# cryscan/bevy-hikari

Hardware: NVIDIA H100
Metric: Mrays/s (higher is better)
Workload: dtype f32

## Files before the change

### bevy_hikari_b200/csrc/context.cu

```cuda
#include <cuda_runtime.h>
#ifndef HK_EMU
#include <cuda.h>
#endif
#include <math.h>
#include <stdio.h>
#include <stdlib.h>
#include <string.h>

#include <algorithm>
#include <array>
#include <set>
#include <string>
#include <unordered_set>
#include <vector>

#include "hikari_b200.h"
#include "hk_kernels.h"
#include "wide_build.h"

#ifndef HK_POOLED_INDIRECT
#define HK_POOLED_INDIRECT 0
#endif

#ifndef HK_WIDE_TRAVERSAL_DEFAULT
// ... 37 lines not shown
    std::vector<hk_node> host_asset_nodes;
    std::vector<uint32_t> host_primitive_vertex_index;
    std::set<std::array<uint32_t, 4>> mesh_range_checked;
    Planes planes{};
    DeviceScene scene{};
    bool scene_ready = false, noise_ready = false;
    bool planes_ready = false;
    TileMap tm_depth[2], tm_q3[2][2];
    TileMap tm_denoise[4][5];
    bool tile_maps_ready = false;
    bool full_frame = true;
    int last_up_w = 0, last_up_h = 0;
    bool last_scaled = false;
    int last_render_w = 0, last_render_h = 0; bool last_smaa = false, last_upscalers = false, last_fsr = false; uint32_t last_number = 0;
    int gbuffer_current = 0;
    uint8_t* noise = nullptr;
    Counters* counters = nullptr;
    SpatialTable* spatial_tables = nullptr;
    SpatialTable spatial_tables_host[2];
    bool count_rays = false, time_passes = false, keep_intermediates = false;
    bool pooled_indirect = HK_POOLED_INDIRECT != 0;
    bool tiled_denoise = true;
    bool tiled_spatial = true;
    int wide_traversal = 0;
    uint32_t wide_tlas_node_count = 0;
    cudaStream_t copy_stream = nullptr;
    cudaEvent_t ev_submitted = nullptr, ev_copied = nullptr;
    bool copy_in_flight = false;
    bool copy_unwaited = false;
    uint2* frame_target = nullptr; uint32_t frame_pitch = 0;
    bool tile_upscalers = false;
    int motion_margin = 0;
    std::vector<void*> frames_owned, frames_opened;
    std::vector<hk_halo_peer*> halo_peers;
    float trace_ms = 0.0f;
    cudaEvent_t ev[4] = {nullptr, nullptr, nullptr, nullptr};
    cudaEvent_t kev[HK_K_COUNT][2] = {};
    int time_only = -1;
    static const int RING = 256;
    cudaEvent_t ring[RING][2] = {};
    uint32_t ring_frames = 0;
    bool ring_hit = false;
    bool kran[HK_K_COUNT] = {};
    hk_frame_stats stats{};
    uint32_t launches = 0;
    std::string error;
// ... 65 lines not shown
    const uint64_t rows = (uint64_t)(b.a1 - b.a0), pitch = (uint64_t)b.AW;
    bool ok = true;
    for (int v = 0; v < 2 && ok; ++v) {
        const uint32_t bh = 16u + 2u * (v ? 10u : 20u), bw = (uint32_t)tile_box_width((int)bh);
        ok = make_tile_map(&ctx->tm_depth[v], ctx->planes.depth, 4, pitch, rows, pitch * 4, bw, bh);
        for (int parity = 0; parity < 2 && ok; ++parity)
            ok = make_tile_map(&ctx->tm_q3[v][parity], ctx->planes.reservoir[(v ? 2 : 6) + parity].q[3], 4, pitch * 4, rows, pitch * 16, bw * 4, bh);
    }
    for (int level = 0; level < 4 && ok; ++level) {
        const uint32_t step = 8u >> level, bh = 16u + 2u * step, bw = (uint32_t)tile_box_width((int)bh);
        ok = make_tile_map(&ctx->tm_denoise[level][0], ctx->planes.dn_geometry, 4, pitch * 4, rows, pitch * 16, bw * 4, bh) &&
             make_tile_map(&ctx->tm_denoise[level][1], ctx->planes.dn_instance, 4, pitch, rows, pitch * 4, bw, bh);
        for (int sgl = 0; sgl < 3 && ok; ++sgl)
            ok = make_tile_map(&ctx->tm_denoise[level][2 + sgl], ctx->planes.dn_internal[level][sgl], 4, pitch * 2, rows, pitch * 8, bw * 2, bh);
    }
    return ok;
}

static int allocate_planes(hk_context* ctx, uint32_t width, uint32_t height, uint32_t col_begin, uint32_t col_end,
                           uint32_t row_begin, uint32_t row_end) {
    if (width == 0 || height == 0 || row_begin >= row_end || row_end > height || col_begin >= col_end || col_end > width)
        return set_error(ctx, HK_ERR_INVALID_ARGUMENT, "bad size or tile rectangle");
    ctx->planes_ready = false;
    ctx->last_render_w = ctx->last_render_h = 0; ctx->last_up_w = ctx->last_up_h = 0; ctx->last_number = 0; ctx->last_scaled = false;
    ctx->last_smaa = ctx->last_upscalers = ctx->last_fsr = false;
    ctx->frame_target = nullptr; ctx->frame_pitch = 0;
    free_list(ctx->allocations);
    ctx->planes = Planes{};
    Band b;
    b.W = (int)width; b.H = (int)height; b.r0 = (int)row_begin; b.r1 = (int)row_end; b.cx0 = (int)col_begin; b.cx1 = (int)col_end;
    const int ghost = GHOST_TEMPORAL + ctx->motion_margin;
    b.a0 = b.r0 - ghost < 0 ? 0 : b.r0 - ghost;
    b.a1 = b.r1 + ghost > b.H ? b.H : b.r1 + ghost;
    b.ax0 = b.cx0 - ghost < 0 ? 0 : b.cx0 - ghost;
    b.ax1 = b.cx1 + ghost > b.W ? b.W : b.cx1 + ghost;
    b.AW = hk_plane_pitch(b.ax1 - b.ax0);
    b.RW = b.W; b.RH = b.H; b.RS = b.AW; b.OW = 2 * b.W; b.OH = 2 * b.H;
    ctx->band = b;
    const size_t n = (size_t)b.AW * (size_t)(b.a1 - b.a0);
    ctx->band_pixels = n;
    ctx->owned_pixels = (size_t)(b.cx1 - b.cx0) * (size_t)(b.r1 - b.r0);
    Planes& p = ctx->planes;
    auto& L = ctx->allocations;
    ctx->full_frame = (b.cx0 == 0 && b.cx1 == b.W && b.r0 == 0 && b.r1 == b.H);
    ctx->gbuffer_current = 0;
    HK_CUDA(alloc_plane(ctx, &p.pos_depth_db[0], n, L));
    HK_CUDA(alloc_plane(ctx, &p.pos_depth_db[1], n, L));
    HK_CUDA(alloc_plane(ctx, &p.velocity_uv_db[0], n, L));
    HK_CUDA(alloc_plane(ctx, &p.velocity_uv_db[1], n, L));
    p.pos_depth = p.pos_depth_db[0];
    p.velocity_uv = p.velocity_uv_db[0];
    HK_CUDA(alloc_plane(ctx, &p.depth, n, L));
    HK_CUDA(alloc_plane(ctx, &p.normal, n, L));
    HK_CUDA(alloc_plane(ctx, &p.depth_gradient, n, L));
    HK_CUDA(alloc_plane(ctx, &p.instance_material, n, L));
    HK_CUDA(alloc_plane(ctx, &p.albedo, n, L));
    HK_CUDA(alloc_plane(ctx, &p.dn_geometry, n, L));
    HK_CUDA(alloc_plane(ctx, &p.dn_instance, n, L));
    for (int i = 0; i < 3; ++i) {
        HK_CUDA(alloc_plane(ctx, &p.render[i], n, L));
        HK_CUDA(alloc_plane(ctx, &p.variance[i], n, L));
        HK_CUDA(alloc_plane(ctx, &p.dn_variance[i], n, L));
        HK_CUDA(alloc_plane(ctx, &p.dn_render[i], n, L));
        for (int l = 0; l < 4; ++l) HK_CUDA(alloc_plane(ctx, &p.dn_internal[l][i], n, L));
    }
    for (int r = 0; r < 10; ++r)
        for (int q = 0; q < 4; ++q) HK_CUDA(alloc_plane(ctx, &p.reservoir[r].q[q], n, L));
    HK_CUDA(alloc_plane(ctx, &p.scatter_key, n, L));
    for (int q = 0; q < 4; ++q) HK_CUDA(alloc_plane(ctx, &p.scatter_value.q[q], n, L));
    HK_CUDA(alloc_plane(ctx, &p.tone_mapped_db[0], ctx->owned_pixels, L));
    HK_CUDA(alloc_plane(ctx, &p.tone_mapped_db[1], ctx->owned_pixels, L));
    p.tone_mapped = p.tone_mapped_db[0];
    p.upscale_output = nullptr; p.upscale_sharpen_output = nullptr; p.taa_output[0] = p.taa_output[1] = nullptr;
    p.tone_ring_db[0] = p.tone_ring_db[1] = nullptr;
    if (!ctx->full_frame && ctx->tile_upscalers) {
// ... 19 lines not shown

int hk_context_create(hk_context** out, int cuda_device, uint32_t width, uint32_t height, uint32_t row_begin, uint32_t row_end,
                      void* cuda_stream) {
    return hk_context_create_tile(out, cuda_device, width, height, 0, width, row_begin, row_end, cuda_stream);
}

int hk_context_create_tile(hk_context** out, int cuda_device, uint32_t width, uint32_t height, uint32_t col_begin, uint32_t col_end,
                           uint32_t row_begin, uint32_t row_end, void* cuda_stream) {
    hk_context* ctx = nullptr;
    if (!out) return set_error(nullptr, HK_ERR_INVALID_ARGUMENT, "out == NULL");
    *out = nullptr;
    int ndev = 0;
    cudaError_t e = cudaGetDeviceCount(&ndev);
    if (e != cudaSuccess || ndev == 0)
        return set_error(nullptr, HK_ERR_CUDA, std::string("no CUDA device: ") + cudaGetErrorString(e) +
                                                   " (this library has no CPU fallback)");
    if (cuda_device < 0 || cuda_device >= ndev) return set_error(nullptr, HK_ERR_INVALID_ARGUMENT, "bad cuda_device");
    HK_CUDA(cudaSetDevice(cuda_device));
    hk_context* c = new hk_context();
    c->device = cuda_device;
    if (const char* e = getenv("HK_TUNE_POOLED_INDIRECT")) c->pooled_indirect = atoi(e) != 0;
    if (const char* e = getenv("HK_TUNE_TILED_SPATIAL")) c->tiled_spatial = atoi(e) != 0;
    if (const char* e = getenv("HK_TUNE_TILED_DENOISE")) c->tiled_denoise = atoi(e) != 0;
    c->wide_traversal = hk_tolerance_build() != 0 ? HK_WIDE_TRAVERSAL_DEFAULT : 0;
    if (const char* e = getenv("HK_TUNE_WIDE_TRAVERSAL")) c->wide_traversal = atoi(e) & 3;
#ifndef HK_EMU
    if (const char* e = getenv("HK_TUNE_PREFER_L1")) { if (atoi(e)) cudaDeviceSetCacheConfig(cudaFuncCachePreferL1); }
#endif
    ctx = c;
    if (cuda_stream) c->stream = reinterpret_cast<cudaStream_t>(cuda_stream);
    else {
        e = cudaStreamCreateWithFlags(&c->stream, cudaStreamNonBlocking);
        if (e != cudaSuccess) { delete c; return set_error(nullptr, HK_ERR_CUDA, cudaGetErrorString(e)); }
        c->own_stream = true;
    }
    int rc = allocate_planes(c, width, height, col_begin, col_end, row_begin, row_end);
    if (rc == HK_OK) {
        void* p = nullptr;
        if (cudaMalloc(&p, sizeof(Counters)) != cudaSuccess) rc = set_error(c, HK_ERR_OUT_OF_MEMORY, "counters");
        else { c->counters = reinterpret_cast<Counters*>(p); cudaMemsetAsync(p, 0, sizeof(Counters), c->stream); }
    }
    if (rc == HK_OK) {
        SpatialTable t[2];
        memset(t, 0, sizeof(t));
        for (int v = 0; v < 2; ++v) {
            const uint32_t count = v ? 8u : 16u;
// ... 568 lines not shown
                                                  "and a motion margin of at least 4 pixels + the per-frame motion");
    if (in->temporal_upscalers && in->fsr1 && in->smaa_tu4x)
        return set_error(ctx, HK_ERR_INVALID_ARGUMENT, "fsr1 and smaa_tu4x are the two variants of one enum (Upscale, lib.rs:475-490)");
    if (in->temporal_upscalers && in->fsr1 && !ctx->full_frame)
        return set_error(ctx, HK_ERR_UNSUPPORTED, "FSR1 needs a full-frame context (no tile)");
    if (in->frame.direct_validate_interval == 0 || in->frame.emissive_validate_interval == 0)
        return set_error(ctx, HK_ERR_INVALID_ARGUMENT, "validate interval must be >= 1");
    if (cudaSetDevice(ctx->device) != cudaSuccess) return set_error(ctx, HK_ERR_CUDA, "cudaSetDevice");
    P.in = *in;
    P.scene = ctx->scene;
    P.planes = ctx->planes;
    P.planes.pos_depth = ctx->planes.pos_depth_db[ctx->gbuffer_current];
    P.planes.velocity_uv = ctx->planes.velocity_uv_db[ctx->gbuffer_current];
    P.planes.tone_mapped = ctx->planes.tone_mapped_db[in->temporal_upscalers ? (in->frame.number % 2u) : 0u];
    ctx->last_upscalers = in->temporal_upscalers != 0;
    P.band = ctx->band;
    P.ratio1 = ratio1 ? 1 : 0;
    P.jitter_sign = ((in->frame.number & 1u) == 0u) ? -1.0f : 1.0f;
    P.ratio_m1 = in->frame.upscale_ratio - 1.0f;
    P.gbuffer_current = ctx->gbuffer_current;
    P.frame_target = ratio1 ? ctx->frame_target : nullptr;
    P.frame_pitch = ctx->frame_pitch;
    P.tile_images = (!ctx->full_frame && in->temporal_upscalers) ? 1 : 0;
    if (!ratio1) {
        const float scale = 1.0f / in->frame.upscale_ratio;
        P.band.RW = (int)ceilf(scale * (float)P.band.W);
        P.band.RH = (int)ceilf(scale * (float)P.band.H);
        P.band.RS = P.band.RW;
    }
    {
        const float scale2 = (1.0f / in->frame.upscale_ratio) * 2.0f;
        P.band.OW = (int)ceilf((float)P.band.W * scale2);
        P.band.OH = (int)ceilf((float)P.band.H * scale2);
    }
    ctx->last_up_w = P.band.OW; ctx->last_up_h = P.band.OH; ctx->last_scaled = !ratio1;
    P.inv_rw = 1.0f / (float)P.band.RW; P.inv_rh = 1.0f / (float)P.band.RH;
    ctx->last_render_w = P.band.RW; ctx->last_render_h = P.band.RH; ctx->last_smaa = in->smaa_tu4x != 0; ctx->last_number = in->frame.number;
    ctx->last_fsr = in->temporal_upscalers && in->fsr1;
    P.counters = ctx->count_rays ? ctx->counters : nullptr;
    P.noise = ctx->noise;
    float s, c;
    hk::sincos_(in->frame.solar_angle, &s, &c);
    P.cos_solar_angle = c;
    P.random_frame = hk::random_float(in->frame.number);
    P.spatial_tables = ctx->spatial_tables;
    return HK_OK;
// ... 35 lines not shown
}

struct KernelTimer {
    hk_context* c; int k;
    KernelTimer(hk_context* ctx, int kernel) : c(ctx), k(kernel) {
        c->launches += 1;
        if (c->time_only >= 0) {
            if (c->time_only == k && c->ring[0][0]) { cudaEventRecord(c->ring[c->ring_frames % hk_context::RING][0], c->stream); c->ring_hit = true; }
        } else if (c->time_passes) { cudaEventRecord(c->kev[k][0], c->stream); c->kran[k] = true; }
    }
    ~KernelTimer() {
        if (c->time_only >= 0) {
            if (c->time_only == k && c->ring[0][0]) cudaEventRecord(c->ring[c->ring_frames % hk_context::RING][1], c->stream);
        } else if (c->time_passes) cudaEventRecord(c->kev[k][1], c->stream);
    }
};

static int run_prepass(hk_context* ctx, KParams& P) {
    ctx->gbuffer_current ^= 1;
    P.gbuffer_current = ctx->gbuffer_current;
    P.planes.pos_depth = ctx->planes.pos_depth_db[ctx->gbuffer_current];
    P.planes.velocity_uv = ctx->planes.velocity_uv_db[ctx->gbuffer_current];
    rows_deferred(ctx, P, GHOST_TEMPORAL + ctx->motion_margin);
    { KernelTimer t(ctx, HK_K_GBUFFER); hk_launch_gbuffer(P, ctx->count_rays, wide_primary(ctx), ctx->stream); }
    return check_launch(ctx);
}
static int ring_of(const KParams& P) { return P.tile_images ? RING_TONE : 0; }
static void launch_spatial(hk_context* ctx, const KParams& P, bool emissive) {
    const int v = emissive ? 1 : 0, parity = 1 - (int)(P.in.frame.number & 1u);
    const bool tiled = ctx->tile_maps_ready && ctx->tiled_spatial;
    hk_launch_spatial(P, emissive, tiled ? &ctx->tm_depth[v] : nullptr, tiled ? &ctx->tm_q3[v][parity] : nullptr, ctx->spatial_tables_host[v], ctx->stream);
}
static const TileMap* denoise_maps(hk_context* ctx, int level) { return (ctx->tile_maps_ready && ctx->tiled_denoise) ? ctx->tm_denoise[level] : nullptr; }
static int run_light(hk_context* ctx, KParams& P) {
    const hk_frame_uniform& f = P.in.frame;
    const int GHOST_SPATIAL = ::GHOST_SPATIAL + ring_of(P);
    rows(ctx, P, GHOST_TEMPORAL + ctx->motion_margin);
    { KernelTimer t(ctx, HK_K_DIRECT); hk_launch_direct(P, false, ctx->count_rays, wide_light(ctx), ctx->stream);
      hk_launch_scatter_resolve(P, 0, ctx->stream); ctx->launches += 1; }
    { KernelTimer t(ctx, HK_K_EMISSIVE); hk_launch_direct(P, true, ctx->count_rays, wide_light(ctx), ctx->stream);
      hk_launch_scatter_resolve(P, 1, ctx->stream); ctx->launches += 1; }
    if (f.emissive_spatial_reuse) { rows(ctx, P, GHOST_SPATIAL); KernelTimer t(ctx, HK_K_EMISSIVE_SPATIAL); launch_spatial(ctx, P, true); }
    rows(ctx, P, GHOST_TEMPORAL + ctx->motion_margin);
    { KernelTimer t(ctx, HK_K_INDIRECT);
      if (ctx->pooled_indirect) hk_launch_indirect_pool(P, f.indirect_bounces >= 2, ctx->count_rays, ctx->stream);
      else hk_launch_indirect(P, f.indirect_bounces >= 2, ctx->count_rays, wide_light(ctx), ctx->stream);
      hk_launch_scatter_resolve(P, 2, ctx->stream); ctx->launches += 1; }
// ... 49 lines not shown
        }
    }
    return check_launch(ctx);
}

int hk_prepass_run(hk_context* ctx, const hk_frame_inputs* in) {
    KParams P; int rc = make_params(ctx, in, P); if (rc) return rc;
    ctx->launches = 0;
    return run_prepass(ctx, P);
}
int hk_import_gbuffer(hk_context* ctx, const hk_gbuffer_desc* g) {
    if (!ctx || !g) return HK_ERR_INVALID_ARGUMENT;
    if (!ctx->planes_ready) return set_error(ctx, HK_ERR_NOT_READY, "per-pixel planes are not allocated (a resize failed)");
    if (!g->position || !g->normal || !g->depth_gradient || !g->instance_material || !g->velocity_uv)
        return set_error(ctx, HK_ERR_INVALID_ARGUMENT, "hk_import_gbuffer: all five planes are required");
    const Band& b = ctx->band;
    const size_t ow = (size_t)(b.cx1 - b.cx0), oh = (size_t)(b.r1 - b.r0);
    const size_t pitch[5] = {g->position_pitch_bytes, g->normal_pitch_bytes, g->depth_gradient_pitch_bytes, g->instance_material_pitch_bytes, g->velocity_uv_pitch_bytes};
    const size_t bpp[5] = {16, 4, 8, 8, 16};
    for (int i = 0; i < 5; ++i)
        if (pitch[i] < ow * bpp[i]) return set_error(ctx, HK_ERR_INVALID_ARGUMENT, "hk_import_gbuffer: a row pitch is smaller than the owned rectangle's row");
    HK_CUDA(cudaSetDevice(ctx->device));
    ctx->gbuffer_current ^= 1;
    Planes& p = ctx->planes;
    const size_t first = (size_t)(b.r0 - b.a0) * (size_t)b.AW + (size_t)(b.cx0 - b.ax0);
    void* dst[5] = {p.pos_depth_db[ctx->gbuffer_current] + first, p.normal + first, p.depth_gradient + first, p.instance_material + first,
                    p.velocity_uv_db[ctx->gbuffer_current] + first};
    const void* src[5] = {g->position, g->normal, g->depth_gradient, g->instance_material, g->velocity_uv};
    for (int i = 0; i < 5; ++i)
        HK_CUDA(cudaMemcpy2DAsync(dst[i], (size_t)b.AW * bpp[i], src[i], pitch[i], ow * bpp[i], oh, cudaMemcpyDeviceToDevice, ctx->stream));
    return HK_OK;
}
int hk_light_run(hk_context* ctx, const hk_frame_inputs* in) {
    KParams P; int rc = make_params(ctx, in, P); if (rc) return rc;
    ctx->launches = 0;
    rows_deferred(ctx, P, GHOST_TEMPORAL + ctx->motion_margin);
    hk_launch_albedo(P, ctx->stream);
    ctx->launches += 1;
    return run_light(ctx, P);
}
int hk_post_process_run(hk_context* ctx, const hk_frame_inputs* in) {
    KParams P; int rc = make_params(ctx, in, P); if (rc) return rc;
    ctx->launches = 0;
    return run_post(ctx, P, false);
}
int hk_run_pass(hk_context* ctx, const hk_frame_inputs* in, int pass, int arg) {
// ... 46 lines not shown
    return HK_OK;
}

int hk_sync(hk_context* ctx) {
    if (!ctx) return HK_ERR_INVALID_ARGUMENT;
    HK_CUDA(cudaSetDevice(ctx->device));
    HK_CUDA(cudaStreamSynchronize(ctx->stream));
    if (ctx->copy_unwaited) { HK_CUDA(cudaEventSynchronize(ctx->ev_copied)); ctx->copy_unwaited = false; }
    return HK_OK;
}

int hk_set_profiling(hk_context* ctx, int count_rays, int time_passes) {
    if (!ctx) return HK_ERR_INVALID_ARGUMENT;
    ctx->count_rays = count_rays != 0;
    ctx->time_passes = time_passes != 0;
    return HK_OK;
}
int hk_set_tuning(hk_context* ctx, int key, int value) {
    if (!ctx) return HK_ERR_INVALID_ARGUMENT;
    switch (key) {
        case HK_TUNE_POOLED_INDIRECT: ctx->pooled_indirect = value != 0; return HK_OK;
        case HK_TUNE_TILED_SPATIAL: ctx->tiled_spatial = value != 0; return HK_OK;
        case HK_TUNE_TILED_DENOISE: ctx->tiled_denoise = value != 0; return HK_OK;
        case HK_TUNE_WIDE_TRAVERSAL:
            if (value < 0 || value > 3 || value == 2) return set_error(ctx, HK_ERR_INVALID_ARGUMENT, "HK_TUNE_WIDE_TRAVERSAL takes 0, 1 or 3");
            ctx->wide_traversal = value; return HK_OK;
        default: return set_error(ctx, HK_ERR_INVALID_ARGUMENT, "unknown tuning key");
    }
}
int hk_set_profiling_kernel(hk_context* ctx, int kernel) {
    if (!ctx || kernel >= HK_K_COUNT) return HK_ERR_INVALID_ARGUMENT;
    HK_CUDA(cudaSetDevice(ctx->device));
    ctx->time_only = kernel < 0 ? -1 : kernel;
    ctx->ring_frames = 0;
    if (kernel >= 0 && !ctx->ring[0][0])
        for (int i = 0; i < hk_context::RING; ++i)
            for (int j = 0; j < 2; ++j) HK_CUDA(cudaEventCreate(&ctx->ring[i][j]));
    return HK_OK;
}
int hk_set_keep_intermediates(hk_context* ctx, int keep) {
    if (!ctx) return HK_ERR_INVALID_ARGUMENT;
    ctx->keep_intermediates = keep != 0;
    return HK_OK;
}

int hk_get_stats(hk_context* ctx, hk_frame_stats* out) {
// ... 140 lines not shown
        }
        const size_t n = (size_t)(rb.cx1 - rb.cx0) * (size_t)(rb.r1 - rb.r0);
        if (bytes != n * 64) return set_error(ctx, HK_ERR_INVALID_ARGUMENT, "size mismatch");
        uint4* tmp = nullptr;
        HK_CUDA(cudaMalloc(reinterpret_cast<void**>(&tmp), bytes));
        const unsigned blocks = (unsigned)((n + 255) / 256);
        cudaError_t e;
        if (to_host) {
            k_gather_reservoir<<<blocks, 256, 0, ctx->stream>>>(ctx->planes.reservoir[which - HK_OUT_RESERVOIR_0], rb, n, tmp);
            e = cudaMemcpyAsync(host, tmp, bytes, cudaMemcpyDeviceToHost, ctx->stream);
        } else {
            e = cudaMemcpyAsync(tmp, host, bytes, cudaMemcpyHostToDevice, ctx->stream);
            k_scatter_reservoir<<<blocks, 256, 0, ctx->stream>>>(ctx->planes.reservoir[which - HK_OUT_RESERVOIR_0], rb, n, tmp);
        }
        cudaError_t e2 = cudaStreamSynchronize(ctx->stream);
        cudaFree(tmp);
        HK_CUDA(e);
        HK_CUDA(e2);
        return HK_OK;
    }
    PlaneView v;
    if (!plane_view(ctx, which, &v)) return set_error(ctx, HK_ERR_INVALID_ARGUMENT, "unknown plane id");
    if (bytes != v.w * v.h * v.bpp) return set_error(ctx, HK_ERR_INVALID_ARGUMENT, "size mismatch");
    if (to_host) HK_CUDA(cudaMemcpy2DAsync(host, v.w * v.bpp, v.ptr, v.pitch * v.bpp, v.w * v.bpp, v.h, cudaMemcpyDeviceToHost, ctx->stream));
    else HK_CUDA(cudaMemcpy2DAsync(v.ptr, v.pitch * v.bpp, host, v.w * v.bpp, v.w * v.bpp, v.h, cudaMemcpyHostToDevice, ctx->stream));
    if (!to_host && which == HK_OUT_GBUFFER_POSITION) {
        KParams P{};
        P.planes = ctx->planes; P.planes.pos_depth = ctx->planes.pos_depth_db[ctx->gbuffer_current]; P.band = ctx->band;
        P.row_lo = ctx->band.r0; P.row_hi = ctx->band.r1; P.col_lo = ctx->band.cx0; P.col_hi = ctx->band.cx1;
        hk_launch_extract_depth(P, ctx->stream);
    }
    HK_CUDA(cudaStreamSynchronize(ctx->stream));
    return HK_OK;
}
int hk_readback(hk_context* ctx, int which, void* host, size_t bytes) { return transfer(ctx, which, host, bytes, true); }

int hk_readback_async(hk_context* ctx, int which, void* pinned_host, size_t bytes) {
    if (!ctx || !pinned_host) return HK_ERR_INVALID_ARGUMENT;
    PlaneView v;
    if ((which != HK_OUT_TONE_MAPPED && which != HK_OUT_UPSCALED && which != HK_OUT_TAA && which != HK_OUT_FSR_SHARPENED) || !plane_view(ctx, which, &v))
        return set_error(ctx, HK_ERR_UNSUPPORTED, "hk_readback_async serves the final images (tone-mapped, upscaled, TAA, FSR-sharpened)");
    if (bytes != v.w * v.h * v.bpp) return set_error(ctx, HK_ERR_INVALID_ARGUMENT, "size mismatch");
    HK_CUDA(cudaSetDevice(ctx->device));
    if (!ctx->copy_stream) {
        HK_CUDA(cudaStreamCreateWithFlags(&ctx->copy_stream, cudaStreamNonBlocking));
        HK_CUDA(cudaEventCreateWithFlags(&ctx->ev_submitted, cudaEventDisableTiming));
// ... 234 lines not shown
```

### bevy_hikari_b200/csrc/hk_device.cuh

```cuda
#pragma once
#include <cuda_runtime.h>
#include <stdint.h>

#include "hikari_b200.h"
#include "hk_math.h"

#ifndef HK_INL_PACK
#define HK_INL_PACK __forceinline__
#endif
#ifndef HK_INL_TRAVERSE
#define HK_INL_TRAVERSE __forceinline__
#endif
#ifndef HK_INL_HITINFO
#define HK_INL_HITINFO __forceinline__
#endif
#ifndef HK_INL_TEXTURE
#define HK_INL_TEXTURE __forceinline__
#endif
#ifndef HK_SURFACE_LOOP
#define HK_SURFACE_LOOP 0
#endif
#ifndef HK_INL_SURFACE
#define HK_INL_SURFACE __forceinline__
#endif
// ... 47 lines not shown
    StagePlan stage;
    const hk_wide_node* wide_tlas;
    const hk_wide_node* wide_blas;
    const uint2* wide_instance;
    const uint32_t* wide_instance_rank;
    const uint32_t* wide_primitive_rank;
    uint32_t wide_tlas_root;
    uint32_t wide_ready;
};

struct ReservoirPlanes {
    uint4* q[4];
};

struct Planes {
    float4* pos_depth;
    uint32_t* normal;
    float2* depth_gradient;
    float2* instance_material;
    float4* velocity_uv;
    float* depth;
    float4* pos_depth_db[2];
    float4* velocity_uv_db[2];
    uint2* albedo;
    uint2* render[3];
    float* variance[3];
    ReservoirPlanes reservoir[10];
    uint32_t* scatter_key;
    ReservoirPlanes scatter_value;
    float4* dn_geometry;
    float* dn_instance;
    uint2* dn_internal[4][3];
    float* dn_variance[3];
    uint2* dn_render[3];
    uint2* tone_mapped;
    uint2* tone_mapped_db[2];
    uint2* tone_ring_db[2];
    uint2* upscale_output;
    uint2* upscale_sharpen_output;
    uint2* taa_output[2];
};

__host__ __device__ inline int hk_plane_pitch(int w) { return (w + 3) & ~3; }

struct Band {
    int W, H;
// ... 14 lines not shown
    float tap_ratio[17][6];
};

struct KParams {
    hk_frame_inputs in;
    DeviceScene scene;
    Planes planes;
    Band band;
    Counters* counters;
    const uint8_t* noise;
    int row_lo, row_hi;
    int col_lo, col_hi;
    float cos_solar_angle;
    float random_frame;
    const SpatialTable* spatial_tables;
    int ratio1;
    float jitter_sign;
    float ratio_m1;
    int gbuffer_current;
    uint2* frame_target;
    uint32_t frame_pitch;
    float inv_rw, inv_rh;
    int tile_images;
};

__device__ __forceinline__ float4 ldg4(const void* p) { return __ldg(reinterpret_cast<const float4*>(p)); }
__device__ __forceinline__ uint4 ldg4u(const void* p) { return __ldg(reinterpret_cast<const uint4*>(p)); }
__device__ __forceinline__ vec3 f4xyz(float4 a) { return v3(a.x, a.y, a.z); }
__device__ __forceinline__ vec4 f4v(float4 a) { return v4(a.x, a.y, a.z, a.w); }
__device__ __forceinline__ float4 vf4(vec4 a) { return make_float4(a.x, a.y, a.z, a.w); }

struct Ray { vec3 origin, direction, inv_direction; };
struct Hit { float u, v, distance; uint32_t instance_index, primitive_index; };
struct HitInfo { vec4 position; vec3 normal; vec2 uv; uint32_t instance_index, material_index; };
struct Surface { vec4 base_color, emissive; float reflectance, metallic, roughness, occlusion; };
struct LightCandidate { vec3 direction; float max_distance, min_distance; uint32_t emissive_instance; float p; };

struct Sample {
    vec4 radiance, random, visible_position;
    vec3 visible_normal;
    uint32_t visible_instance;
    vec4 sample_position;
    vec3 sample_normal;
};
struct Reservoir { Sample s; float count, lifetime, w, w_sum, w2_sum; };

// ... 678 lines not shown
#endif
#ifndef HK_MINB_GBUFFER
#define HK_MINB_GBUFFER 8
#endif
#ifndef HK_MINB_INDIRECT_WIDE
#define HK_MINB_INDIRECT_WIDE 6
#endif
#ifndef HK_MINB_DIRECT_WIDE
#define HK_MINB_DIRECT_WIDE 6
#endif
#ifndef HK_MINB_DENOISE
#define HK_MINB_DENOISE 8
#endif
#ifndef HK_MINB_SPATIAL
#define HK_MINB_SPATIAL 8
#endif
__device__ __forceinline__ void tile_pixel(int& x, int& y, const KParams& P) {
    int lane = threadIdx.x & 31, warp = threadIdx.x >> 5;
    x = P.col_lo + blockIdx.x * TILE_W + (warp & 1) * 8 + (lane & 7);
    y = P.row_lo + blockIdx.y * TILE_H + (warp >> 1) * 4 + (lane >> 3);
}
__device__ __forceinline__ bool tile_active(const KParams& P, int x, int y) { return x < P.col_hi && y < P.row_hi; }

}
```

### bevy_hikari_b200/csrc/kernels_light.cu

```cuda
#include "hk_device.cuh"
#include "hk_wide.cuh"
#include "hk_kernels.h"

#ifndef HK_NO_TEXTURE_VARIANT
#define HK_NO_TEXTURE_VARIANT 1
#endif
#ifndef HK_NOVAL_VARIANT
#define HK_NOVAL_VARIANT 1
#endif

namespace hkd {

template <bool COUNT>
__device__ __forceinline__ void flush_counters(const KParams& P, uint32_t primary, uint32_t tlas, uint32_t blas) {
    if (!COUNT || P.counters == nullptr) return;
    for (int o = 16; o > 0; o >>= 1) {
        primary += __shfl_xor_sync(0xffffffffu, primary, o);
        tlas += __shfl_xor_sync(0xffffffffu, tlas, o);
        blas += __shfl_xor_sync(0xffffffffu, blas, o);
    }
    if ((threadIdx.x & 31) == 0) {
        if (primary) atomicAdd(&P.counters->primary, (unsigned long long)primary);
        if (tlas) atomicAdd(&P.counters->tlas, (unsigned long long)tlas);
        if (blas) atomicAdd(&P.counters->blas, (unsigned long long)blas);
// ... 101 lines not shown
            vec4 cy = mul(view_proj, v4(ry.origin + ry.direction * ty, 1.0f));
            vec2 grad = v2(cx.z / cx.w - depth, cy.z / cy.w - depth);
            vec3 previous_world_position = world_position;
            if (sc.instance_moved != nullptr && __ldg(&sc.instance_moved[hit.instance_index]) != 0u) {
                const float4* pm = sc.previous_models + 4u * (size_t)hit.instance_index;
                mat4 previous_model;
                for (int c = 0; c < 4; ++c) previous_model.c[c] = f4v(ldg4(pm + c));
                vec3 local_position = f4xyz(pa) + hit.u * (f4xyz(pb) - f4xyz(pa)) + hit.v * (f4xyz(pc) - f4xyz(pa));
                previous_world_position = xyz(mul(previous_model, v4(local_position, 1.0f)));
            }
            vec4 pclip = mul(load_mat4(P.in.previous_view.view_proj), v4(previous_world_position, 1.0f));
            vec2 uva = v2(clip.x, clip.y) / clip.w; uva = (uva + 1.0f) * 0.5f; uva.y = 1.0f - uva.y;
            vec2 uvb = v2(pclip.x, pclip.y) / pclip.w; uvb = (uvb + 1.0f) * 0.5f; uvb.y = 1.0f - uvb.y;
            vec2 velocity = uva - uvb;
            uint32_t packed_normal = pack4x8snorm(v4(world_normal, 1.0f));
            P.planes.pos_depth[idx] = make_float4(world_position.x, world_position.y, world_position.z, depth);
            P.planes.depth[idx] = depth;
            P.planes.normal[idx] = packed_normal;
            P.planes.depth_gradient[idx] = make_float2(grad.x, grad.y);
            P.planes.instance_material[idx] = make_float2((float)hit.instance_index + 0.5f, (float)material + 0.5f);
            P.planes.velocity_uv[idx] = make_float4(velocity.x, velocity.y, tex_uv.x, tex_uv.y);
            uvec2 alb; alb.x = 0u; alb.y = 0u;
            if (!(depth < F32_EPSILON)) {
                ShadeEnv env = make_env(P);
                vec3 normal = xyz(unpack4x8snorm(packed_normal));
                Surface surface = retreive_surface(sc, f32_to_u32((float)material + 0.5f), tex_uv);
                vec3 view_direction = calculate_view(env, world_position);
                alb = pack_rgba16f(v4(env_brdf(view_direction, normal, surface), 1.0f));
            }
            P.planes.albedo[idx] = make_uint2(alb.x, alb.y);
        }
    }
    if (!band_owned(P.band, x, y)) n_primary = 0;
    flush_counters<COUNT>(P, n_primary, 0u, 0u);
}

__global__ void __launch_bounds__(CTA_THREADS) k_albedo(const __grid_constant__ KParams P) {
    int x, y;
    tile_pixel(x, y, P);
    if (!tile_active(P, x, y)) return;
    const size_t idx = band_index(P.band, x, y);
    float4 pd = P.planes.pos_depth[idx];
    P.planes.depth[idx] = pd.w;
    if (pd.w < F32_EPSILON) { P.planes.albedo[idx] = make_uint2(0u, 0u); return; }
    ShadeEnv env = make_env(P);
    vec3 normal = xyz(unpack4x8snorm(P.planes.normal[idx]));
// ... 440 lines not shown
```

### bevy_hikari_b200/csrc/kernels_post.cu

```cuda
#include "hk_tile.cuh"
#include "hk_kernels.h"

#ifndef HK_DENOISE_BRANCHFREE
#define HK_DENOISE_BRANCHFREE 1
#endif

namespace hkd {

__device__ __forceinline__ vec4 load16(const uint2* plane, size_t i) {
    uint2 u = plane[i];
    uvec2 w; w.x = u.x; w.y = u.y;
    return unpack_rgba16f(w);
}
__device__ __forceinline__ void store16(uint2* plane, size_t i, vec4 v) {
    uvec2 w = pack_rgba16f(v);
    plane[i] = make_uint2(w.x, w.y);
}
__device__ __forceinline__ void store_final(const KParams& P, int x, int y, vec4 color) {
    uvec2 w = pack_rgba16f(color);
    const uint2 bits = make_uint2(w.x, w.y);
    if (P.tile_images) P.planes.tone_ring_db[P.in.frame.number % 2u][band_index(P.band, x, y)] = bits;
    if (!band_owned(P.band, x, y)) return;
    P.planes.tone_mapped[owned_index(P.band, x, y)] = bits;
    if (P.frame_target) P.frame_target[(size_t)y * P.frame_pitch + (size_t)x] = bits;
// ... 233 lines not shown
}

template <int LEVEL> struct DenoiseTile {
    static constexpr int STEP = 8 >> LEVEL;
    static constexpr int BH = POOL_TILE_H + 2 * STEP;
    static constexpr int BW = tile_box_width(POOL_TILE_W + 2 * STEP);
    static constexpr size_t GEO = ((size_t)BW * BH * 16 + 127) & ~(size_t)127, INST = ((size_t)BW * BH * 4 + 127) & ~(size_t)127, SIG = ((size_t)BW * BH * 8 + 127) & ~(size_t)127;
    static constexpr size_t SMEM_BYTES = GEO + INST + 3 * SIG + 16;
};
struct DenoiseMaps { TileMap geometry, instance, signal[3]; };

template <int LEVEL, bool FUSE_TONE_MAPPING>
__global__ void __launch_bounds__(POOL_THREADS, 4) kc_denoise(const __grid_constant__ KParams P, const __grid_constant__ DenoiseMaps M, int signals, int keep_denoised) {
    using DT = DenoiseTile<LEVEL>;
    constexpr int STEP = DT::STEP, BW = DT::BW, BH = DT::BH;
    HK_DYNAMIC_SMEM(smem);
    float4* s_geo = reinterpret_cast<float4*>(smem);
    float* s_inst = reinterpret_cast<float*>(smem + DT::GEO);
    uint2* s_sig[3] = {reinterpret_cast<uint2*>(smem + DT::GEO + DT::INST), reinterpret_cast<uint2*>(smem + DT::GEO + DT::INST + DT::SIG),
                       reinterpret_cast<uint2*>(smem + DT::GEO + DT::INST + 2 * DT::SIG)};
    uint64_t* s_bar = reinterpret_cast<uint64_t*>(smem + DT::GEO + DT::INST + 3 * DT::SIG);
    const int px = tile_origin_x(P.col_lo + (int)blockIdx.x * POOL_TILE_W - STEP - P.band.ax0);
    const int tx0 = px + P.band.ax0, ty0 = P.row_lo + (int)blockIdx.y * POOL_TILE_H - STEP;
    if (threadIdx.x == 0) {
        mbar_init(s_bar, 1u);
        mbar_expect_tx(s_bar, (uint32_t)((size_t)BW * BH * (20 + 8 * (size_t)signals)));
        const int py = ty0 - P.band.a0;
        tile_load_2d(s_geo, &M.geometry, 4 * px, py, s_bar);
        tile_load_2d(s_inst, &M.instance, px, py, s_bar);
        for (int sgl = 0; sgl < signals; ++sgl) tile_load_2d(s_sig[sgl], &M.signal[sgl], 2 * px, py, s_bar);
        mbar_complete_emulated(s_bar);
    }
    __syncthreads();
    int x, y;
    pool_pixel(x, y, P);
    const bool in_launch = tile_active(P, x, y);
    const size_t idx = in_launch ? render_index(P.band, x, y) : 0;
    float2 dg = make_float2(0.0f, 0.0f);
    float dn_var[3] = {0.0f, 0.0f, 0.0f};
    uint2 albedo_bits = make_uint2(0u, 0u);
    if (in_launch) {
        dg = __ldg(&P.planes.depth_gradient[idx]);
#pragma unroll
        for (int sgl = 0; sgl < 3; ++sgl) if (sgl < signals) dn_var[sgl] = __ldg(&P.planes.dn_variance[sgl][idx]);
        if (LEVEL == 3) albedo_bits = __ldg(&P.planes.albedo[idx]);
    }
    mbar_wait(s_bar, 0u);
    if (!in_launch) return;
    const int cx = x - tx0, cy = y - ty0;
    const float4 geometry = s_geo[cy * BW + cx];
    const float depth = geometry.w;
    vec4 result[3];
    result[0] = result[1] = result[2] = v4(0.0f);
    if (!(depth < F32_EPSILON)) {
        const vec2 depth_gradient = v2(dg.x, dg.y);
        const vec3 normal = f4xyz(geometry);
        const float instance = s_inst[cy * BW + cx];
        SignalAcc acc[3];
#pragma unroll
        for (int sgl = 0; sgl < 3; ++sgl) {
            if (sgl >= signals) continue;
            SignalAcc& a = acc[sgl];
            a.lum_denominator = 4.0f * pow025(dn_var[sgl]) + 0.001f;
            const uint2 cb = s_sig[sgl][cy * BW + cx];
            uvec2 cq; cq.x = cb.x; cq.y = cb.y;
            a.irradiance = xyz(unpack_rgba16f(cq));
            a.sum_irradiance = a.irradiance * kernel_at(P, 1, 1);
            a.sum_w = kernel_at(P, 1, 1);
            if (bad3(a.irradiance)) { a.irradiance = v3(0.0f); a.sum_irradiance = v3(0.0f); a.sum_w = 0.0f; }
            a.lum = luminance(a.irradiance);
            a.ff_moment_1 = 0.0f; a.ff_moment_2 = 0.0f; a.ff_count = 0.0f;
        }
        const int OX[8] = {-1, 0, 1, -1, 1, -1, 0, 1};
// ... 199 lines not shown
```

### bevy_hikari_b200/plugin.py

```python
import ctypes as C
import os

import numpy as np

from . import _ffi
from . import layout as L
from ._ffi import Settings, check, host_lib, lib

TAA_JASMINE, TAA_NONE = 0, 1
TUNE_POOLED_INDIRECT, TUNE_TILED_SPATIAL, TUNE_TILED_DENOISE, TUNE_WIDE_TRAVERSAL = 1, 2, 3, 4
UPSCALE_FSR1, UPSCALE_SMAA_TU4X = 0, 1
NOISE_PATH = os.path.join(os.path.dirname(os.path.dirname(os.path.abspath(__file__))), "data", "noise_rgba8_64x64x16.bin")


def graph_name():
    return host_lib().hikari_graph_name().decode()


def HikariSettings(**overrides):
    s = Settings()
    host_lib().hikari_settings_default(C.byref(s))
    for k, v in overrides.items():
        if k == "clear_color":
            s.clear_color[:] = list(v)
        elif not hasattr(s, k):
            raise AttributeError(f"HikariSettings has no field {k}")
        else:
            setattr(s, k, v)
    return s


def make_frame_inputs(settings, frame_counter, view, previous_view, lights, temporal_upscalers=False):
    out = L.FrameInputs()
# ... 370 lines not shown
```

### include/hikari_b200.h

```cpp
#ifndef HIKARI_B200_H
#define HIKARI_B200_H
#include <stddef.h>
#include <stdint.h>
#include "hk_layout.h"

#ifdef __cplusplus
extern "C" {
#endif

#define HK_OK 0
#define HK_ERR_INVALID_ARGUMENT (-1)
#define HK_ERR_CUDA (-2)
#define HK_ERR_NOT_READY (-3)
#define HK_ERR_OUT_OF_MEMORY (-4)
#define HK_ERR_UNSUPPORTED (-5)

typedef struct hk_context hk_context;

typedef struct hk_texture_desc {
    const uint8_t* rgba8;
    uint32_t width, height;
    uint32_t address_mode_u;
    uint32_t address_mode_v;
    uint32_t filter_linear;
// ... 134 lines not shown
int hk_context_set_motion_margin(hk_context* ctx, uint32_t pixels);
int hk_halo_pull(hk_context* dst, hk_context* src);
int hk_context_enable_tile_upscalers(hk_context* ctx, int enabled);
typedef struct hk_halo_descriptor {
    uint8_t plane_handles[44][64];
    int32_t has_images;
    int32_t frame[2];
    int32_t allocated[4];
    int32_t owned[4];
} hk_halo_descriptor;
typedef struct hk_halo_peer hk_halo_peer;
int hk_halo_export(hk_context* ctx, hk_halo_descriptor* out);
int hk_halo_import(hk_context* ctx, const hk_halo_descriptor* remote, hk_halo_peer** out);
int hk_halo_pull_peer(hk_context* ctx, hk_halo_peer* peer);

int hk_set_frame_target(hk_context* ctx, void* frame_device_ptr, uint32_t pitch_pixels);
int hk_frame_alloc(hk_context* ctx, void** device_ptr, uint8_t ipc_handle[64]);
int hk_frame_open(hk_context* ctx, const uint8_t ipc_handle[64], void** device_ptr);
int hk_frame_read(hk_context* ctx, const void* frame_device_ptr, void* host, size_t bytes);

int hk_trace_rays(hk_context* ctx, const hk_ray* rays, size_t n, hk_hit* hits);
int hk_set_profiling(hk_context* ctx, int count_rays, int time_passes);
int hk_set_profiling_kernel(hk_context* ctx, int kernel);
enum { HK_TUNE_POOLED_INDIRECT = 1, HK_TUNE_TILED_SPATIAL = 2, HK_TUNE_TILED_DENOISE = 3, HK_TUNE_WIDE_TRAVERSAL = 4 };
int hk_set_tuning(hk_context* ctx, int key, int value);
int hk_set_keep_intermediates(hk_context* ctx, int keep);
int hk_get_stats(hk_context* ctx, hk_frame_stats* out);
int hk_band_rows(hk_context* ctx, uint32_t* alloc_row_begin, uint32_t* alloc_row_end);
int hk_tile_rect(hk_context* ctx, uint32_t allocated[4], uint32_t owned[4]);

const char* hk_last_error(hk_context* ctx);
const char* hk_version(void);

#ifdef __cplusplus
}
#endif
#endif
```

### rust/hikari-b200-sys/src/lib.rs

```rust
#![no_std]
#![allow(non_camel_case_types, non_upper_case_globals)]

pub const HK_OK: ::core::ffi::c_int = 0;
pub const HK_ERR_INVALID_ARGUMENT: ::core::ffi::c_int = -1;
pub const HK_ERR_CUDA: ::core::ffi::c_int = -2;
pub const HK_ERR_NOT_READY: ::core::ffi::c_int = -3;
pub const HK_ERR_OUT_OF_MEMORY: ::core::ffi::c_int = -4;
pub const HK_ERR_UNSUPPORTED: ::core::ffi::c_int = -5;
pub const HK_OUT_TONE_MAPPED: ::core::ffi::c_int = 0;
pub const HK_OUT_RENDER_DIRECT: ::core::ffi::c_int = 1;
pub const HK_OUT_RENDER_EMISSIVE: ::core::ffi::c_int = 2;
pub const HK_OUT_RENDER_INDIRECT: ::core::ffi::c_int = 3;
pub const HK_OUT_VARIANCE_DIRECT: ::core::ffi::c_int = 4;
pub const HK_OUT_VARIANCE_EMISSIVE: ::core::ffi::c_int = 5;
pub const HK_OUT_VARIANCE_INDIRECT: ::core::ffi::c_int = 6;
pub const HK_OUT_ALBEDO: ::core::ffi::c_int = 7;
pub const HK_OUT_DENOISED_DIRECT: ::core::ffi::c_int = 8;
pub const HK_OUT_DENOISED_EMISSIVE: ::core::ffi::c_int = 9;
pub const HK_OUT_DENOISED_INDIRECT: ::core::ffi::c_int = 10;
pub const HK_OUT_UPSCALED: ::core::ffi::c_int = 11;
pub const HK_OUT_TAA: ::core::ffi::c_int = 12;
pub const HK_OUT_FSR_SHARPENED: ::core::ffi::c_int = 13;
pub const HK_OUT_GBUFFER_POSITION: ::core::ffi::c_int = 16;
pub const HK_OUT_GBUFFER_NORMAL: ::core::ffi::c_int = 17;
// ... 8 lines not shown
pub const HK_K_INDIRECT: ::core::ffi::c_int = 4;
pub const HK_K_INDIRECT_SPATIAL: ::core::ffi::c_int = 5;
pub const HK_K_DEMODULATION: ::core::ffi::c_int = 6;
pub const HK_K_DENOISE_0: ::core::ffi::c_int = 7;
pub const HK_K_DENOISE_1: ::core::ffi::c_int = 8;
pub const HK_K_DENOISE_2: ::core::ffi::c_int = 9;
pub const HK_K_DENOISE_3: ::core::ffi::c_int = 10;
pub const HK_K_TONE_MAPPING: ::core::ffi::c_int = 11;
pub const HK_K_SMAA_TU4X: ::core::ffi::c_int = 12;
pub const HK_K_TAA: ::core::ffi::c_int = 13;
pub const HK_K_FSR1: ::core::ffi::c_int = 14;
pub const HK_K_COUNT: ::core::ffi::c_int = 15;
pub const HK_K_TRACE_RAYS: ::core::ffi::c_int = 15;
pub const HK_SCENE_INSTANCES: ::core::ffi::c_int = 0;
pub const HK_SCENE_INSTANCE_NODES: ::core::ffi::c_int = 1;
pub const HK_SCENE_EMISSIVES: ::core::ffi::c_int = 2;
pub const HK_SCENE_EMISSIVE_NODES: ::core::ffi::c_int = 3;
pub const HK_SCENE_PREVIOUS_MODELS: ::core::ffi::c_int = 4;
pub const HK_SCENE_INSTANCE_MOVED: ::core::ffi::c_int = 5;
pub const HK_TUNE_POOLED_INDIRECT: ::core::ffi::c_int = 1;
pub const HK_TUNE_TILED_SPATIAL: ::core::ffi::c_int = 2;
pub const HK_TUNE_TILED_DENOISE: ::core::ffi::c_int = 3;
pub const HK_TUNE_WIDE_TRAVERSAL: ::core::ffi::c_int = 4;

#[repr(C)] pub struct hk_context { _private: [u8; 0] }
#[repr(C)] pub struct hk_halo_peer { _private: [u8; 0] }

#[repr(C)]
#[derive(Clone, Copy)]
pub struct hk_node {
    pub min: [f32; 3],
    pub entry_index: u32,
    pub max: [f32; 3],
    pub exit_index: u32,
}
#[repr(C)]
#[derive(Clone, Copy)]
pub struct hk_primitive_vertex {
    pub position: [f32; 3],
    pub index: u32,
}
#[repr(C)]
#[derive(Clone, Copy)]
pub struct hk_primitive {
    pub vertices: [hk_primitive_vertex; 3],
}
// ... 303 lines not shown
```

Measured before the change: 1823.

## Skip denoise tile staging for tiles without any surface pixels

The gbuffer kernel now stamps a per-tile surface map with a generation counter wherever a pixel has geometry. The pooled denoise kernel checks this map with a block-wide OR and skips the TMA tile load and per-pixel loads for all-background tiles, using zero geometry instead. The map is invalidated on gbuffer import or plane upload. This trades an extra global write per surface pixel and a block sync for less memory traffic on empty tiles. Correctness depends on background pixels producing the same result from zero inputs.

```diff
diff --git a/bevy_hikari_b200/csrc/context.cu b/bevy_hikari_b200/csrc/context.cu
--- a/bevy_hikari_b200/csrc/context.cu
+++ b/bevy_hikari_b200/csrc/context.cu
@@ -83,6 +83,9 @@
     bool pooled_indirect = HK_POOLED_INDIRECT != 0;
     bool tiled_denoise = true;
     bool tiled_spatial = true;
+    bool skip_background_tiles = true;
+    bool tile_surface_valid = false;
+    uint32_t surface_generation = 0;
     int wide_traversal = 0;
     uint32_t wide_tlas_node_count = 0;
     cudaStream_t copy_stream = nullptr;
@@ -194,6 +197,7 @@
     if (width == 0 || height == 0 || row_begin >= row_end || row_end > height || col_begin >= col_end || col_end > width)
         return set_error(ctx, HK_ERR_INVALID_ARGUMENT, "bad size or tile rectangle");
     ctx->planes_ready = false;
+    ctx->tile_surface_valid = false;
     ctx->last_render_w = ctx->last_render_h = 0; ctx->last_up_w = ctx->last_up_h = 0; ctx->last_number = 0; ctx->last_scaled = false;
     ctx->last_smaa = ctx->last_upscalers = ctx->last_fsr = false;
     ctx->frame_target = nullptr; ctx->frame_pitch = 0;
@@ -223,6 +227,7 @@
     p.pos_depth = p.pos_depth_db[0];
     p.velocity_uv = p.velocity_uv_db[0];
     HK_CUDA(alloc_plane(ctx, &p.depth, n, L));
+    HK_CUDA(alloc_plane(ctx, &p.tile_surface, (size_t)surface_cells_x(b.W) * (size_t)surface_cells_y(b.H), L));
     HK_CUDA(alloc_plane(ctx, &p.normal, n, L));
     HK_CUDA(alloc_plane(ctx, &p.depth_gradient, n, L));
     HK_CUDA(alloc_plane(ctx, &p.instance_material, n, L));
@@ -288,6 +293,7 @@
     if (const char* e = getenv("HK_TUNE_POOLED_INDIRECT")) c->pooled_indirect = atoi(e) != 0;
     if (const char* e = getenv("HK_TUNE_TILED_SPATIAL")) c->tiled_spatial = atoi(e) != 0;
     if (const char* e = getenv("HK_TUNE_TILED_DENOISE")) c->tiled_denoise = atoi(e) != 0;
+    if (const char* e = getenv("HK_TUNE_SKIP_BACKGROUND_TILES")) c->skip_background_tiles = atoi(e) != 0;
     c->wide_traversal = hk_tolerance_build() != 0 ? HK_WIDE_TRAVERSAL_DEFAULT : 0;
     if (const char* e = getenv("HK_TUNE_WIDE_TRAVERSAL")) c->wide_traversal = atoi(e) & 3;
 #ifndef HK_EMU
@@ -902,6 +908,8 @@
     P.frame_target = ratio1 ? ctx->frame_target : nullptr;
     P.frame_pitch = ctx->frame_pitch;
     P.tile_images = (!ctx->full_frame && in->temporal_upscalers) ? 1 : 0;
+    P.surface_generation = ctx->surface_generation;
+    P.skip_background = (ctx->skip_background_tiles && ctx->tile_surface_valid && ratio1) ? 1 : 0;
     if (!ratio1) {
         const float scale = 1.0f / in->frame.upscale_ratio;
         P.band.RW = (int)ceilf(scale * (float)P.band.W);
@@ -983,7 +991,10 @@
     P.planes.pos_depth = ctx->planes.pos_depth_db[ctx->gbuffer_current];
     P.planes.velocity_uv = ctx->planes.velocity_uv_db[ctx->gbuffer_current];
     rows_deferred(ctx, P, GHOST_TEMPORAL + ctx->motion_margin);
+    P.surface_generation = ctx->surface_generation += 1u;
     { KernelTimer t(ctx, HK_K_GBUFFER); hk_launch_gbuffer(P, ctx->count_rays, wide_primary(ctx), ctx->stream); }
+    ctx->tile_surface_valid = true;
+    P.skip_background = (ctx->skip_background_tiles && P.ratio1) ? 1 : 0;
     return check_launch(ctx);
 }
 static int ring_of(const KParams& P) { return P.tile_images ? RING_TONE : 0; }
@@ -1079,6 +1090,7 @@
         if (pitch[i] < ow * bpp[i]) return set_error(ctx, HK_ERR_INVALID_ARGUMENT, "hk_import_gbuffer: a row pitch is smaller than the owned rectangle's row");
     HK_CUDA(cudaSetDevice(ctx->device));
     ctx->gbuffer_current ^= 1;
+    ctx->tile_surface_valid = false;
     Planes& p = ctx->planes;
     const size_t first = (size_t)(b.r0 - b.a0) * (size_t)b.AW + (size_t)(b.cx0 - b.ax0);
     void* dst[5] = {p.pos_depth_db[ctx->gbuffer_current] + first, p.normal + first, p.depth_gradient + first, p.instance_material + first,
@@ -1171,6 +1183,7 @@
         case HK_TUNE_POOLED_INDIRECT: ctx->pooled_indirect = value != 0; return HK_OK;
         case HK_TUNE_TILED_SPATIAL: ctx->tiled_spatial = value != 0; return HK_OK;
         case HK_TUNE_TILED_DENOISE: ctx->tiled_denoise = value != 0; return HK_OK;
+        case HK_TUNE_SKIP_BACKGROUND_TILES: ctx->skip_background_tiles = value != 0; return HK_OK;
         case HK_TUNE_WIDE_TRAVERSAL:
             if (value < 0 || value > 3 || value == 2) return set_error(ctx, HK_ERR_INVALID_ARGUMENT, "HK_TUNE_WIDE_TRAVERSAL takes 0, 1 or 3");
             ctx->wide_traversal = value; return HK_OK;
@@ -1357,6 +1370,7 @@
     PlaneView v;
     if (!plane_view(ctx, which, &v)) return set_error(ctx, HK_ERR_INVALID_ARGUMENT, "unknown plane id");
     if (bytes != v.w * v.h * v.bpp) return set_error(ctx, HK_ERR_INVALID_ARGUMENT, "size mismatch");
+    if (!to_host) ctx->tile_surface_valid = false;
     if (to_host) HK_CUDA(cudaMemcpy2DAsync(host, v.w * v.bpp, v.ptr, v.pitch * v.bpp, v.w * v.bpp, v.h, cudaMemcpyDeviceToHost, ctx->stream));
     else HK_CUDA(cudaMemcpy2DAsync(v.ptr, v.pitch * v.bpp, host, v.w * v.bpp, v.w * v.bpp, v.h, cudaMemcpyHostToDevice, ctx->stream));
     if (!to_host && which == HK_OUT_GBUFFER_POSITION) {
diff --git a/bevy_hikari_b200/csrc/hk_device.cuh b/bevy_hikari_b200/csrc/hk_device.cuh
--- a/bevy_hikari_b200/csrc/hk_device.cuh
+++ b/bevy_hikari_b200/csrc/hk_device.cuh
@@ -93,6 +93,7 @@
     float* depth;
     float4* pos_depth_db[2];
     float4* velocity_uv_db[2];
+    uint32_t* tile_surface;
     uint2* albedo;
     uint2* render[3];
     float* variance[3];
@@ -153,6 +154,8 @@
     uint32_t frame_pitch;
     float inv_rw, inv_rh;
     int tile_images;
+    uint32_t surface_generation;
+    int skip_background;
 };
 
 __device__ __forceinline__ float4 ldg4(const void* p) { return __ldg(reinterpret_cast<const float4*>(p)); }
@@ -877,4 +880,13 @@
 }
 __device__ __forceinline__ bool tile_active(const KParams& P, int x, int y) { return x < P.col_hi && y < P.row_hi; }
 
-}
+__host__ __device__ inline int surface_cells_x(int width) { return (width + TILE_W - 1) / TILE_W; }
+__host__ __device__ inline int surface_cells_y(int height) { return (height + TILE_H - 1) / TILE_H; }
+__device__ __forceinline__ size_t surface_cell(const Band& b, int x, int y) {
+    return (size_t)(y / TILE_H) * (size_t)surface_cells_x(b.W) + (size_t)(x / TILE_W);
+}
+__device__ __forceinline__ bool tile_has_surface(const KParams& P, bool in_launch, int x, int y) {
+    return __syncthreads_or(in_launch && __ldg(&P.planes.tile_surface[surface_cell(P.band, x, y)]) == P.surface_generation) != 0;
+}
+
+}
diff --git a/bevy_hikari_b200/csrc/kernels_light.cu b/bevy_hikari_b200/csrc/kernels_light.cu
--- a/bevy_hikari_b200/csrc/kernels_light.cu
+++ b/bevy_hikari_b200/csrc/kernels_light.cu
@@ -147,6 +147,7 @@
             P.planes.velocity_uv[idx] = make_float4(velocity.x, velocity.y, tex_uv.x, tex_uv.y);
             uvec2 alb; alb.x = 0u; alb.y = 0u;
             if (!(depth < F32_EPSILON)) {
+                P.planes.tile_surface[surface_cell(P.band, x, y)] = P.surface_generation;
                 ShadeEnv env = make_env(P);
                 vec3 normal = xyz(unpack4x8snorm(packed_normal));
                 Surface surface = retreive_surface(sc, f32_to_u32((float)material + 0.5f), tex_uv);
diff --git a/bevy_hikari_b200/csrc/kernels_post.cu b/bevy_hikari_b200/csrc/kernels_post.cu
--- a/bevy_hikari_b200/csrc/kernels_post.cu
+++ b/bevy_hikari_b200/csrc/kernels_post.cu
@@ -279,8 +279,14 @@
     uint64_t* s_bar = reinterpret_cast<uint64_t*>(smem + DT::GEO + DT::INST + 3 * DT::SIG);
     const int px = tile_origin_x(P.col_lo + (int)blockIdx.x * POOL_TILE_W - STEP - P.band.ax0);
     const int tx0 = px + P.band.ax0, ty0 = P.row_lo + (int)blockIdx.y * POOL_TILE_H - STEP;
-    if (threadIdx.x == 0) {
-        mbar_init(s_bar, 1u);
+    int x, y;
+    pool_pixel(x, y, P);
+    const bool in_launch = tile_active(P, x, y);
+    if (threadIdx.x == 0) mbar_init(s_bar, 1u);
+    bool staged = true;
+    if (P.skip_background) staged = tile_has_surface(P, in_launch, x, y);
+    else __syncthreads();
+    if (threadIdx.x == 0 && staged) {
         mbar_expect_tx(s_bar, (uint32_t)((size_t)BW * BH * (20 + 8 * (size_t)signals)));
         const int py = ty0 - P.band.a0;
         tile_load_2d(s_geo, &M.geometry, 4 * px, py, s_bar);
@@ -288,24 +294,20 @@
         for (int sgl = 0; sgl < signals; ++sgl) tile_load_2d(s_sig[sgl], &M.signal[sgl], 2 * px, py, s_bar);
         mbar_complete_emulated(s_bar);
     }
-    __syncthreads();
-    int x, y;
-    pool_pixel(x, y, P);
-    const bool in_launch = tile_active(P, x, y);
     const size_t idx = in_launch ? render_index(P.band, x, y) : 0;
     float2 dg = make_float2(0.0f, 0.0f);
     float dn_var[3] = {0.0f, 0.0f, 0.0f};
     uint2 albedo_bits = make_uint2(0u, 0u);
-    if (in_launch) {
+    if (in_launch && staged) {
         dg = __ldg(&P.planes.depth_gradient[idx]);
 #pragma unroll
         for (int sgl = 0; sgl < 3; ++sgl) if (sgl < signals) dn_var[sgl] = __ldg(&P.planes.dn_variance[sgl][idx]);
         if (LEVEL == 3) albedo_bits = __ldg(&P.planes.albedo[idx]);
     }
-    mbar_wait(s_bar, 0u);
+    if (staged) mbar_wait(s_bar, 0u);
     if (!in_launch) return;
     const int cx = x - tx0, cy = y - ty0;
-    const float4 geometry = s_geo[cy * BW + cx];
+    const float4 geometry = staged ? s_geo[cy * BW + cx] : make_float4(0.0f, 0.0f, 0.0f, 0.0f);
     const float depth = geometry.w;
     vec4 result[3];
     result[0] = result[1] = result[2] = v4(0.0f);
diff --git a/bevy_hikari_b200/plugin.py b/bevy_hikari_b200/plugin.py
--- a/bevy_hikari_b200/plugin.py
+++ b/bevy_hikari_b200/plugin.py
@@ -8,7 +8,7 @@
 from ._ffi import Settings, check, host_lib, lib
 
 TAA_JASMINE, TAA_NONE = 0, 1
-TUNE_POOLED_INDIRECT, TUNE_TILED_SPATIAL, TUNE_TILED_DENOISE, TUNE_WIDE_TRAVERSAL = 1, 2, 3, 4
+TUNE_POOLED_INDIRECT, TUNE_TILED_SPATIAL, TUNE_TILED_DENOISE, TUNE_WIDE_TRAVERSAL, TUNE_SKIP_BACKGROUND_TILES = 1, 2, 3, 4, 5
 UPSCALE_FSR1, UPSCALE_SMAA_TU4X = 0, 1
 NOISE_PATH = os.path.join(os.path.dirname(os.path.dirname(os.path.abspath(__file__))), "data", "noise_rgba8_64x64x16.bin")
 
diff --git a/include/hikari_b200.h b/include/hikari_b200.h
--- a/include/hikari_b200.h
+++ b/include/hikari_b200.h
@@ -180,7 +180,7 @@
 int hk_trace_rays(hk_context* ctx, const hk_ray* rays, size_t n, hk_hit* hits);
 int hk_set_profiling(hk_context* ctx, int count_rays, int time_passes);
 int hk_set_profiling_kernel(hk_context* ctx, int kernel);
-enum { HK_TUNE_POOLED_INDIRECT = 1, HK_TUNE_TILED_SPATIAL = 2, HK_TUNE_TILED_DENOISE = 3, HK_TUNE_WIDE_TRAVERSAL = 4 };
+enum { HK_TUNE_POOLED_INDIRECT = 1, HK_TUNE_TILED_SPATIAL = 2, HK_TUNE_TILED_DENOISE = 3, HK_TUNE_WIDE_TRAVERSAL = 4, HK_TUNE_SKIP_BACKGROUND_TILES = 5 };
 int hk_set_tuning(hk_context* ctx, int key, int value);
 int hk_set_keep_intermediates(hk_context* ctx, int keep);
 int hk_get_stats(hk_context* ctx, hk_frame_stats* out);
diff --git a/rust/hikari-b200-sys/src/lib.rs b/rust/hikari-b200-sys/src/lib.rs
--- a/rust/hikari-b200-sys/src/lib.rs
+++ b/rust/hikari-b200-sys/src/lib.rs
@@ -54,6 +54,7 @@
 pub const HK_TUNE_TILED_SPATIAL: ::core::ffi::c_int = 2;
 pub const HK_TUNE_TILED_DENOISE: ::core::ffi::c_int = 3;
 pub const HK_TUNE_WIDE_TRAVERSAL: ::core::ffi::c_int = 4;
+pub const HK_TUNE_SKIP_BACKGROUND_TILES: ::core::ffi::c_int = 5;
 
 #[repr(C)] pub struct hk_context { _private: [u8; 0] }
 #[repr(C)] pub struct hk_halo_peer { _private: [u8; 0] }
```

Measured after the change: 1865, median of 6. +2.3%, better.
